# Boese0601/MagicDance

Hardware: NVIDIA H100
Metric: denoise-steps/sec @512x512 50-step DDIM (higher is better)
Workload: dtype f16

## Files before the change

magicdance_b200/csrc/attention.cu:

```cuda
#include <stdlib.h>

#include <type_traits>

#include "common.cuh"

namespace mdb {

constexpr int kBQ = 128;

template <int D, int BKV, int STAGES>
struct AttnCfg {
  static constexpr int kDkChunks = (D + 63) / 64;
  static constexpr int kDV = (D + 15) / 16 * 16;
  static constexpr int kKSteps = kDV / 16;
  static constexpr int kQBytes = kDkChunks * kBQ * 128;
  static constexpr int kKBytes = kDkChunks * BKV * 128;
  static constexpr int kVBytes = kDV * 128;
  static constexpr int kStageBytes = kKBytes + kVBytes;
  static constexpr int kSmem = kQBytes + STAGES * kStageBytes + 1024;
  static_assert(BKV == 64, "one 128-byte swizzle row of keys per V^T tile");
  static_assert(kVBytes % 1024 == 0 && kKBytes % 1024 == 0, "stage tiles start on swizzle-atom boundaries");
};

struct AttnKParams {
  CUtensorMap tmQ, tmK0, tmV0, tmK1, tmV1;
  __half* out;
  long long ldo;
  int nq, n0, n1;
  int kv0_batches, kv1_batches;
  int ldv0_batch, ldv1_batch;
  int bank_batches;
  float scale_log2;
};
struct AttnLseKParams : AttnKParams {
  float* lse;
};

template <int D, int BKV, int STAGES, int MINB, bool LSE = false>
__global__ void __launch_bounds__(kWsThreads, MINB)
    attn_wg_kernel(const __grid_constant__ std::conditional_t<LSE, AttnLseKParams, AttnKParams> p) {
  using C = AttnCfg<D, BKV, STAGES>;
  extern __shared__ uint8_t smem_raw[];
  __shared__ __align__(8) uint64_t q_bar;
  __shared__ __align__(8) uint64_t kv_full[STAGES], kv_empty[STAGES];

  uint8_t* sQ = align1024(smem_raw);
  uint8_t* sKV = sQ + C::kQBytes;

  const int warp = threadIdx.x >> 5;
  const int lane = threadIdx.x & 31;
  const int q0 = blockIdx.x * kBQ;
  const int head = blockIdx.y;
  const int b = blockIdx.z;
  const int t0 = (p.n0 + BKV - 1) / BKV;
  const int t1 = (b < p.bank_batches && p.n1 > 0) ? (p.n1 + BKV - 1) / BKV : 0;
  const int n_tiles = t0 + t1;

  pdl_launch_dependents();
  if (warp == kProducerWarp && lane == 0) {
    tma_prefetch_desc(&p.tmQ);
    tma_prefetch_desc(&p.tmK0);
    tma_prefetch_desc(&p.tmV0);
    mbar_init(&q_bar, 1);
    ring_init<STAGES>(kv_full, kv_empty, 1);
    fence_barrier_init();
  }
  __syncthreads();
  pdl_wait();

  if (warp == kProducerWarp) {
    if (lane == 0) {
      mbar_expect_tx(&q_bar, C::kQBytes);
      for (int dc = 0; dc < C::kDkChunks; ++dc)
        tma_load_3d(sQ + dc * (kBQ * 128), &p.tmQ, &q_bar, dc * 64, head, b * p.nq + q0);
      for (int j = 0; j < n_tiles; ++j) {
        const bool src1 = j >= t0;
        const int key0 = (src1 ? (j - t0) : j) * BKV;
        const CUtensorMap* tk = src1 ? &p.tmK1 : &p.tmK0;
        const CUtensorMap* tv = src1 ? &p.tmV1 : &p.tmV0;
        const int nsrc = src1 ? p.n1 : p.n0;
        const int kvb = src1 ? (p.kv1_batches > 1 ? b : 0) : (p.kv0_batches > 1 ? b : 0);
        const int ldvb = src1 ? p.ldv1_batch : p.ldv0_batch;
        const int s = ring_acquire<STAGES>(kv_empty, j);
        mbar_expect_tx(&kv_full[s], C::kStageBytes);
        uint8_t* sk = sKV + s * C::kStageBytes;
        uint8_t* sv = sk + C::kKBytes;
        for (int dc = 0; dc < C::kDkChunks; ++dc)
          tma_load_3d(sk + dc * (BKV * 128), tk, &kv_full[s], dc * 64, head, kvb * nsrc + key0);
        tma_load_2d(sv, tv, &kv_full[s], kvb * ldvb + key0, head * D);
      }
    }
  } else {
    const int wg = warp >> 2;
    const uint32_t q_addr = smem_u32(sQ) + wg * (64 * 128);
    const int cq = 2 * (lane & 3);
    float o[C::kDV / 2];
#pragma unroll
    for (int i = 0; i < C::kDV / 2; ++i) o[i] = 0.f;
    float m_run[2] = {-INFINITY, -INFINITY};
    float l_run[2] = {0.f, 0.f};
    mbar_wait(&q_bar, 0);

    for (int j = 0; j < n_tiles; ++j) {
      const bool src1 = j >= t0;
      const int key0 = (src1 ? (j - t0) : j) * BKV;
      const int valid = min(BKV, (src1 ? p.n1 : p.n0) - key0);
      const int s = ring_wait_full<STAGES>(kv_full, j);
      const uint32_t k_addr = smem_u32(sKV + s * C::kStageBytes);
      const uint32_t v_addr = k_addr + C::kKBytes;

      float sc[BKV / 2];
      wgmma_fence();
#pragma unroll
      for (int ks = 0; ks < C::kKSteps; ++ks) {
        const int dc = ks >> 2, kk = ks & 3;
        const uint64_t da = wgmma_desc_k_sw128(q_addr + dc * (kBQ * 128)) + 2 * kk;
        const uint64_t db = wgmma_desc_k_sw128(k_addr + dc * (BKV * 128)) + 2 * kk;
        wgmma_ss<BKV>(sc, da, db, ks != 0 ? 1u : 0u);
      }
      wgmma_commit();
      wgmma_wait<0>();
      wgmma_fence_regs(sc);

      if (valid < BKV) {
#pragma unroll
        for (int i = 0; i < BKV / 2; ++i)
          if (8 * (i >> 2) + cq + (i & 1) >= valid) sc[i] = -INFINITY;
      }
      float mx[2] = {-INFINITY, -INFINITY};
#pragma unroll
      for (int i = 0; i < BKV / 2; ++i) mx[(i >> 1) & 1] = fmaxf(mx[(i >> 1) & 1], sc[i]);
      float alpha[2], neg_m[2];
#pragma unroll
      for (int h = 0; h < 2; ++h) {
        mx[h] = fmaxf(mx[h], __shfl_xor_sync(0xffffffffu, mx[h], 1));
        mx[h] = fmaxf(mx[h], __shfl_xor_sync(0xffffffffu, mx[h], 2));
        const float m_new = fmaxf(m_run[h], mx[h] * p.scale_log2);
        alpha[h] = ex2_approx(m_run[h] - m_new);
        m_run[h] = m_new;
        neg_m[h] = -m_new;
      }
      float ls[2] = {0.f, 0.f};
      uint32_t pa[BKV / 16][4];
#pragma unroll
      for (int i = 0; i < BKV / 2; i += 2) {
        const int h = (i >> 1) & 1;
        const float e0 = ex2_approx(fmaf(sc[i], p.scale_log2, neg_m[h]));
        const float e1 = ex2_approx(fmaf(sc[i + 1], p.scale_log2, neg_m[h]));
        ls[h] += e0 + e1;
        pa[i >> 3][(i >> 1) & 3] = pack_half2(e0, e1);
      }
#pragma unroll
      for (int h = 0; h < 2; ++h) l_run[h] = fmaf(l_run[h], alpha[h], ls[h]);
#pragma unroll
      for (int i = 0; i < C::kDV / 2; ++i) o[i] *= alpha[(i >> 1) & 1];

      wgmma_fence();
#pragma unroll
      for (int kk = 0; kk < BKV / 16; ++kk)
        wgmma_rs<C::kDV>(o, pa[kk], wgmma_desc_k_sw128(v_addr) + 2 * kk, 1u);
      wgmma_commit();
      wgmma_wait<0>();
      wgmma_fence_regs(o);
      mbar_arrive(&kv_empty[s]);
    }

    float inv_l[2], l_row[2];
#pragma unroll
    for (int h = 0; h < 2; ++h) {
      float l = l_run[h];
      l += __shfl_xor_sync(0xffffffffu, l, 1);
      l += __shfl_xor_sync(0xffffffffu, l, 2);
      inv_l[h] = 1.0f / l;
      l_row[h] = l;
    }
    const int r = wg * 64 + (warp & 3) * 16 + (lane >> 2);
    if constexpr (LSE) {
      if ((lane & 3) == 0) {
#pragma unroll
        for (int h = 0; h < 2; ++h) {
          const int q = q0 + r + 8 * h;
          if (q < p.nq)
            p.lse[(static_cast<long long>(b) * gridDim.y + head) * p.nq + q] =
                (m_run[h] + log2f(l_row[h])) * 0.6931471805599453f;
        }
      }
    }
#pragma unroll
    for (int h = 0; h < 2; ++h) {
      const int q = q0 + r + 8 * h;
      if (q < p.nq) {
        __half* op = p.out + (static_cast<long long>(b) * p.nq + q) * p.ldo + head * D + cq;
#pragma unroll
        for (int c8 = 0; c8 < D / 8; ++c8)
          *reinterpret_cast<uint32_t*>(op + 8 * c8) =
              pack_half2(o[4 * c8 + 2 * h] * inv_l[h], o[4 * c8 + 2 * h + 1] * inv_l[h]);
      }
    }
  }
}

static int g_attn40_2q_min_ctas = 512;
int get_attn_tuning() { return g_attn40_2q_min_ctas; }
void set_attn_tuning(int v) { g_attn40_2q_min_ctas = v; }

template <int D, int BKV, int STAGES, int MINB, bool LSE = false, typename P>
static int launch_attn(const P& kp, dim3 grid, cudaStream_t st) {
  using C = AttnCfg<D, BKV, STAGES>;
  static_assert(MINB == 1 || C::kSmem <= 113 * 1024, "two CTAs per SM must fit");
  constexpr auto kern = attn_wg_kernel<D, BKV, STAGES, MINB, LSE>;
  if (int rc = set_max_dyn_smem<kern>(C::kSmem)) return rc;
  MDB_CHECK_CUDA(launch_pdl(kern, grid, dim3(kWsThreads), C::kSmem, st, kp));
  count_launch();
  return MDB_OK;
}

template <int D, int BKV>
static int build_and_launch(const mdb_attn_desc* a, float* lse, cudaStream_t st) {
  constexpr int kDV = AttnCfg<D, BKV, 1>::kDV;
  AttnKParams kp;
  memset(&kp, 0, sizeof(kp));
  const int hd = a->heads * a->d;
  int rc;
  if ((rc = tmap_heads(&kp.tmQ, a->q, a->d, a->heads, (uint64_t)a->batch * a->nq, a->ldq, kBQ))) return rc;
  auto mk_kv = [&](const void* k, long long ldk, const void* vt, long long ldvt, int n, int nb, int ldvb,
                   CUtensorMap* tk, CUtensorMap* tv) -> int {
    int r = tmap_heads(tk, k, a->d, a->heads, (uint64_t)nb * n, ldk, BKV);
    if (r) return r;
    return tmap_rows(tv, vt, (uint64_t)nb * ldvb, hd, ldvt, 64, kDV);
  };
  if ((rc = mk_kv(a->k0, a->ldk0, a->vt0, a->ldvt0, a->n0, a->kv0_batches, a->ldv0_batch, &kp.tmK0, &kp.tmV0))) return rc;
  if (a->n1 > 0) {
    if ((rc = mk_kv(a->k1, a->ldk1, a->vt1, a->ldvt1, a->n1, a->kv1_batches, a->ldv1_batch, &kp.tmK1, &kp.tmV1)))
      return rc;
  }
  kp.out = static_cast<__half*>(a->out);
  kp.ldo = a->ldo;
  kp.nq = a->nq;
  kp.n0 = a->n0;
  kp.n1 = a->n1;
  kp.kv0_batches = a->kv0_batches;
  kp.kv1_batches = a->kv1_batches;
  kp.ldv0_batch = a->ldv0_batch;
  kp.ldv1_batch = a->ldv1_batch;
  kp.bank_batches = a->n1 > 0 ? a->bank_batches : 0;
  kp.scale_log2 = a->scale * 1.4426950408889634f;
  dim3 grid((a->nq + kBQ - 1) / kBQ, a->heads, a->batch);
  if (lse != nullptr) {
    AttnLseKParams lp;
    memset(&lp, 0, sizeof(lp));
    static_cast<AttnKParams&>(lp) = kp;
    lp.lse = lse;
    if constexpr (D == 40) {
      const long long ctas = (long long)grid.x * grid.y * grid.z;
      if (ctas >= (long long)g_attn40_2q_min_ctas) return launch_attn<D, BKV, 3, 2, true>(lp, grid, st);
    }
    return launch_attn<D, BKV, (D == 160 ? 2 : 4), 1, true>(lp, grid, st);
  }
  if constexpr (D == 40) {
    const long long ctas = (long long)grid.x * grid.y * grid.z;
    if (ctas >= (long long)g_attn40_2q_min_ctas) return launch_attn<D, BKV, 3, 2>(kp, grid, st);
  }
  return launch_attn<D, BKV, (D == 160 ? 2 : 4), 1>(kp, grid, st);
}

static int attention_entry(const mdb_attn_desc* a, float* lse, cudaStream_t st) {
  switch (a->d) {
    case 40:
      return build_and_launch<40, 64>(a, lse, st);
    case 80:
      return build_and_launch<80, 64>(a, lse, st);
    case 160:
      return build_and_launch<160, 64>(a, lse, st);
    default:
      set_error("mdb_attention_f16: head dim %d not supported (40, 80, 160)", a->d);
      return MDB_ERR_UNSUPPORTED;
  }
}

int attention_check_desc(const mdb_attn_desc* a) {
  MDB_REQUIRE(a != nullptr, "mdb_attention_f16: null descriptor");
  MDB_REQUIRE(a->q && a->k0 && a->vt0 && a->out, "mdb_attention_f16: null operand");
  MDB_REQUIRE(a->batch > 0 && a->heads > 0 && a->nq > 0 && a->n0 > 0 && a->n1 >= 0,
              "mdb_attention_f16: bad shape");
  MDB_REQUIRE(a->n1 == 0 || (a->k1 && a->vt1), "mdb_attention_f16: n1 > 0 needs k1/vt1");
  MDB_REQUIRE(a->kv0_batches == 1 || a->kv0_batches == a->batch, "mdb_attention_f16: kv0_batches must be 1 or batch");
  MDB_REQUIRE(a->n1 == 0 || a->kv1_batches == 1 || a->kv1_batches >= a->bank_batches,
              "mdb_attention_f16: kv1_batches must be 1 or cover bank_batches");
  MDB_REQUIRE(a->ldv0_batch >= a->n0 && a->ldv0_batch % 8 == 0, "mdb_attention_f16: ldv0_batch must be >= n0 and %% 8");
  MDB_REQUIRE(a->ldo % 8 == 0 && (reinterpret_cast<uintptr_t>(a->out) & 15) == 0, "mdb_attention_f16: out alignment");
  return MDB_OK;
}

}

using namespace mdb;

extern "C" int mdb_attention_f16(const mdb_attn_desc* a, mdb_stream_t stream) {
  const int rc = attention_check_desc(a);
  if (rc) return rc;
  return attention_entry(a, nullptr, static_cast<cudaStream_t>(stream));
}

extern "C" int mdb_attention_lse_f16(const mdb_attn_desc* a, float* lse, mdb_stream_t stream) {
  const int rc = attention_check_desc(a);
  if (rc) return rc;
  MDB_REQUIRE(lse != nullptr, "mdb_attention_lse_f16: null lse");
  return attention_entry(a, lse, static_cast<cudaStream_t>(stream));
}
```

magicdance_b200/csrc/common.cuh:

```cuda
#pragma once

#include <cuda.h>
#include <cuda_fp16.h>
#include <cuda_runtime.h>
#include <cudaTypedefs.h>
#include <stdint.h>
#include <stdio.h>
#include <string.h>

#include "../../include/magicdance_b200.h"
#include "wgmma.cuh"

namespace mdb {

void set_error(const char* fmt, ...);

#define MDB_CHECK_CUDA(expr)                                                                     \
  do {                                                                                           \
    cudaError_t _e = (expr);                                                                     \
    if (_e != cudaSuccess) {                                                                     \
      mdb::set_error("%s:%d: %s failed: %s", __FILE__, __LINE__, #expr, cudaGetErrorString(_e)); \
      return MDB_ERR_CUDA;                                                                       \
    }                                                                                            \
  } while (0)

#define MDB_REQUIRE(cond, ...)      \
  do {                              \
    if (!(cond)) {                  \
      mdb::set_error(__VA_ARGS__);  \
      return MDB_ERR_INVALID;       \
    }                               \
  } while (0)

void count_launch(int n = 1);
int get_gemm_tuning(int key);
void set_gemm_tuning(int key, int value);
int get_attn_tuning();
void set_attn_tuning(int v);

constexpr int kNumSms = 132;

int tmap_rows(CUtensorMap* out, const void* base, uint64_t inner, uint64_t rows, long long ld, uint32_t box_inner,
              uint32_t box_rows);
int tmap_heads(CUtensorMap* out, const void* base, int d, int heads, uint64_t tokens, long long ld,
               uint32_t box_tokens);
int tmap_nhwc(CUtensorMap* out, const void* base, int c, int w, int h, int nb, long long ld, const uint32_t box[4],
              int cs);

enum { kBoxOk, kBoxWideRows, kBoxRowsPerTile, kBoxImagesPerTile, kBoxTooLarge };
int pixel_box(int ho, int wo, int cs, int rows, bool fwd, uint32_t box[4]);

#ifdef __CUDACC__

bool pdl_enabled();
template <typename... KArgs, typename... Args>
inline cudaError_t launch_pdl_cluster2(void (*kernel)(KArgs...), dim3 grid, dim3 block, size_t smem,
                                       cudaStream_t stream, unsigned cluster_x, unsigned cluster_z, Args&&... args) {
  cudaLaunchConfig_t cfg;
  memset(&cfg, 0, sizeof(cfg));
  cfg.gridDim = grid;
  cfg.blockDim = block;
  cfg.dynamicSmemBytes = smem;
  cfg.stream = stream;
  cudaLaunchAttribute attr[2];
  int n = 0;
  if (cluster_z > 1 || cluster_x > 1) {
    attr[n].id = cudaLaunchAttributeClusterDimension;
    attr[n].val.clusterDim.x = cluster_x;
    attr[n].val.clusterDim.y = 1;
    attr[n].val.clusterDim.z = cluster_z;
    ++n;
  }
  if (pdl_enabled()) {
    attr[n].id = cudaLaunchAttributeProgrammaticStreamSerialization;
    attr[n].val.programmaticStreamSerializationAllowed = 1;
    ++n;
  }
  cfg.attrs = attr;
  cfg.numAttrs = n;
  return cudaLaunchKernelEx(&cfg, kernel, static_cast<KArgs>(args)...);
}
template <typename... KArgs, typename... Args>
inline cudaError_t launch_pdl_cluster(void (*kernel)(KArgs...), dim3 grid, dim3 block, size_t smem,
                                      cudaStream_t stream, unsigned cluster_z, Args&&... args) {
  return launch_pdl_cluster2(kernel, grid, block, smem, stream, 1u, cluster_z, static_cast<Args&&>(args)...);
}
template <typename... KArgs, typename... Args>
inline cudaError_t launch_pdl(void (*kernel)(KArgs...), dim3 grid, dim3 block, size_t smem, cudaStream_t stream,
                              Args&&... args) {
  return launch_pdl_cluster2(kernel, grid, block, smem, stream, 1u, 1u, static_cast<Args&&>(args)...);
}
template <auto Kernel>
inline int set_max_dyn_smem(int bytes) {
  static bool done = false;
  if (!done) {
    MDB_CHECK_CUDA(cudaFuncSetAttribute(Kernel, cudaFuncAttributeMaxDynamicSharedMemorySize, bytes));
    done = true;
  }
  return MDB_OK;
}

__device__ __forceinline__ uint32_t smem_u32(const void* p) {
  return static_cast<uint32_t>(__cvta_generic_to_shared(p));
}

__device__ __forceinline__ bool elect_one() {
  uint32_t pred = 0;
  asm volatile(
      "{\n\t.reg .pred P;\n\t"
      "elect.sync _|P, 0xffffffff;\n\t"
      "selp.u32 %0, 1, 0, P;\n\t}"
      : "=r"(pred));
  return pred != 0;
}

__device__ __forceinline__ void pdl_launch_dependents() { asm volatile("griddepcontrol.launch_dependents;" ::: "memory"); }
__device__ __forceinline__ void pdl_wait() { asm volatile("griddepcontrol.wait;" ::: "memory"); }

__device__ __forceinline__ void mbar_init(uint64_t* bar, uint32_t count) {
  asm volatile("mbarrier.init.shared::cta.b64 [%0], %1;" ::"r"(smem_u32(bar)), "r"(count));
}
__device__ __forceinline__ void fence_barrier_init() {
  asm volatile("fence.mbarrier_init.release.cluster;" ::: "memory");
}
__device__ __forceinline__ void mbar_expect_tx(uint64_t* bar, uint32_t bytes) {
  asm volatile("mbarrier.arrive.expect_tx.shared::cta.b64 _, [%0], %1;" ::"r"(smem_u32(bar)), "r"(bytes)
               : "memory");
}
__device__ __forceinline__ void mbar_arrive(uint64_t* bar) {
  asm volatile("mbarrier.arrive.shared::cta.b64 _, [%0];" ::"r"(smem_u32(bar)) : "memory");
}
__device__ __forceinline__ void mbar_wait(uint64_t* bar, uint32_t parity) {
  uint32_t addr = smem_u32(bar);
  asm volatile(
      "{\n\t.reg .pred P1;\n\t"
      "WAIT_LOOP:\n\t"
      "mbarrier.try_wait.parity.shared::cta.b64 P1, [%0], %1;\n\t"
      "@P1 bra DONE;\n\t"
      "bra WAIT_LOOP;\n\t"
      "DONE:\n\t}"
      ::"r"(addr), "r"(parity)
      : "memory");
}

constexpr int kConsumers = 256;
constexpr int kProducerWarp = kConsumers / 32;
constexpr int kWsThreads = kConsumers + 32;

__device__ __forceinline__ uint8_t* align1024(uint8_t* p) {
  return reinterpret_cast<uint8_t*>((reinterpret_cast<uintptr_t>(p) + 1023) & ~uintptr_t(1023));
}

template <int S>
__device__ __forceinline__ void ring_init(uint64_t* full, uint64_t* empty, uint32_t full_count) {
  for (int s = 0; s < S; ++s) {
    mbar_init(&full[s], full_count);
    mbar_init(&empty[s], kConsumers);
  }
}
template <int S>
__device__ __forceinline__ int ring_acquire(uint64_t* empty, int it) {
  const int s = it % S;
  mbar_wait(&empty[s], ((it / S) & 1) ^ 1);
  return s;
}
template <int S>
__device__ __forceinline__ int ring_wait_full(uint64_t* full, int it) {
  const int s = it % S;
  mbar_wait(&full[s], (it / S) & 1);
  return s;
}

__device__ __forceinline__ void tma_prefetch_desc(const CUtensorMap* m) {
  asm volatile("prefetch.tensormap [%0];" ::"l"(reinterpret_cast<uint64_t>(m)) : "memory");
}
__device__ __forceinline__ void tma_load_2d(void* dst, const CUtensorMap* m, uint64_t* bar, int c0, int c1) {
  asm volatile(
      "cp.async.bulk.tensor.2d.shared::cluster.global.tile.mbarrier::complete_tx::bytes [%0], [%1, {%3, %4}], [%2];"
      ::"r"(smem_u32(dst)), "l"(reinterpret_cast<uint64_t>(m)), "r"(smem_u32(bar)), "r"(c0), "r"(c1)
      : "memory");
}
__device__ __forceinline__ void tma_load_3d(void* dst, const CUtensorMap* m, uint64_t* bar, int c0, int c1, int c2) {
  asm volatile(
      "cp.async.bulk.tensor.3d.shared::cluster.global.tile.mbarrier::complete_tx::bytes [%0], [%1, {%3, %4, %5}], [%2];"
      ::"r"(smem_u32(dst)), "l"(reinterpret_cast<uint64_t>(m)), "r"(smem_u32(bar)), "r"(c0), "r"(c1), "r"(c2)
      : "memory");
}
__device__ __forceinline__ void tma_load_4d(void* dst, const CUtensorMap* m, uint64_t* bar, int c0, int c1, int c2,
                                            int c3) {
  asm volatile(
      "cp.async.bulk.tensor.4d.shared::cluster.global.tile.mbarrier::complete_tx::bytes [%0], [%1, {%3, %4, %5, %6}], [%2];"
      ::"r"(smem_u32(dst)), "l"(reinterpret_cast<uint64_t>(m)), "r"(smem_u32(bar)), "r"(c0), "r"(c1), "r"(c2), "r"(c3)
      : "memory");
}

__device__ __forceinline__ uint32_t cluster_ctarank() {
  uint32_t r;
  asm volatile("mov.u32 %0, %%cluster_ctarank;" : "=r"(r));
  return r;
}
__device__ __forceinline__ void cluster_sync_all() {
  asm volatile("barrier.cluster.arrive.release.aligned;" ::: "memory");
  asm volatile("barrier.cluster.wait.acquire.aligned;" ::: "memory");
}
__device__ __forceinline__ uint32_t dsmem_map(uint32_t local_smem_addr, uint32_t rank) {
  uint32_t a;
  asm volatile("mapa.shared::cluster.u32 %0, %1, %2;" : "=r"(a) : "r"(local_smem_addr), "r"(rank));
  return a;
}
__device__ __forceinline__ float4 dsmem_ld_f4(uint32_t cluster_addr) {
  float4 v;
  asm volatile("ld.shared::cluster.v4.f32 {%0, %1, %2, %3}, [%4];"
               : "=f"(v.x), "=f"(v.y), "=f"(v.z), "=f"(v.w)
               : "r"(cluster_addr));
  return v;
}

__device__ __forceinline__ void fence_proxy_async_smem() {
  asm volatile("fence.proxy.async.shared::cta;" ::: "memory");
}

__device__ __forceinline__ uint64_t wgmma_desc_k_sw128(uint32_t smem_addr) {
  uint64_t d = 0;
  d |= static_cast<uint64_t>((smem_addr & 0x3FFFF) >> 4);
  d |= static_cast<uint64_t>(1) << 16;
  d |= static_cast<uint64_t>(1024 >> 4) << 32;
  d |= static_cast<uint64_t>(1) << 62;
  return d;
}
__device__ __forceinline__ uint64_t wgmma_desc_mn_sw128(uint32_t smem_addr, uint32_t chunk_bytes) {
  uint64_t d = 0;
  d |= static_cast<uint64_t>((smem_addr & 0x3FFFF) >> 4);
  d |= static_cast<uint64_t>((chunk_bytes >> 4) & 0x3FFF) << 16;
  d |= static_cast<uint64_t>(1024 >> 4) << 32;
  d |= static_cast<uint64_t>(1) << 62;
  return d;
}
__device__ __forceinline__ void wgmma_fence() { asm volatile("wgmma.fence.sync.aligned;" ::: "memory"); }
__device__ __forceinline__ void wgmma_commit() { asm volatile("wgmma.commit_group.sync.aligned;" ::: "memory"); }
template <int N>
__device__ __forceinline__ void wgmma_wait() { asm volatile("wgmma.wait_group.sync.aligned %0;" ::"n"(N) : "memory"); }
template <int R>
__device__ __forceinline__ void wgmma_fence_regs(float (&d)[R]) {
#pragma unroll
  for (int i = 0; i < R; ++i) asm volatile("" : "+f"(d[i])::"memory");
}
__device__ __forceinline__ void named_bar_sync(int id, int threads) {
  asm volatile("bar.sync %0, %1;" ::"r"(id), "r"(threads) : "memory");
}

__device__ __forceinline__ uint32_t pack_half2(float a, float b) {
  __half2 h = __floats2half2_rn(a, b);
  return *reinterpret_cast<uint32_t*>(&h);
}

__device__ __forceinline__ float ex2_approx(float x) {
  float y;
  asm("ex2.approx.ftz.f32 %0, %1;" : "=f"(y) : "f"(x));
  return y;
}
__device__ __forceinline__ float silu_f(float x) { return x / (1.0f + __expf(-x)); }
__device__ __forceinline__ float gelu_erf_f(float x) { return 0.5f * x * (1.0f + erff(x * 0.70710678118654752f)); }
__device__ __forceinline__ float dsilu(float x) {
  const float s = 1.0f / (1.0f + __expf(-x));
  return s * (1.0f + x * (1.0f - s));
}
__device__ __forceinline__ float dgelu_erf(float x) {
  return 0.5f * (1.0f + erff(x * 0.70710678118654752f)) + x * 0.39894228040143268f * __expf(-0.5f * x * x);
}

struct GbOut {
  void* p;
  long long ld;
  int f32, acc;
};

__device__ __forceinline__ void gb_store2(const GbOut& o, long long row, int col, float v0, float v1) {
  if (o.p == nullptr) return;
  if (o.f32) {
    float2* d = reinterpret_cast<float2*>(static_cast<float*>(o.p) + row * o.ld + col);
    if (o.acc) {
      const float2 x = *d;
      v0 += x.x;
      v1 += x.y;
    }
    *d = make_float2(v0, v1);
  } else {
    __half2* d = reinterpret_cast<__half2*>(static_cast<__half*>(o.p) + row * o.ld + col);
    if (o.acc) {
      const float2 x = __half22float2(*d);
      v0 += x.x;
      v1 += x.y;
    }
    *d = __floats2half2_rn(v0, v1);
  }
}
#endif

inline GbOut gb_out(void* p, long long ld, int dtype, int acc) {
  GbOut o;
  o.p = p;
  o.ld = ld;
  o.f32 = dtype == MDB_DTYPE_F32;
  o.acc = acc != 0;
  return o;
}

int launch_colsum_finalize(const float* ws, int n, int segs, int parts, float* out, long long stride, int acc,
                           cudaStream_t st);

}
```

Before: 89.98.

## Add warp-specialized FA3-style pipelined attention kernel for head dim 40

Adds a dedicated head-dim-40 attention kernel with one TMA producer warpgroup and three MMA consumer warpgroups. It uses 128-key tiles, register reallocation via setmaxnreg, and ping-pong named barriers so one warpgroup's QK/PV wgmma overlaps another's softmax. The next tile's QK is issued alongside the previous tile's PV. The kernel is the default path for d=40 whenever there are more than 128 keys, and the tuning knob is repurposed (negative values select the old kernel). It aims to hide softmax latency and raise tensor-core utilization, at the cost of more code, a large register budget, and one CTA per SM.

```diff
diff --git a/magicdance_b200/csrc/attention.cu b/magicdance_b200/csrc/attention.cu
--- a/magicdance_b200/csrc/attention.cu
+++ b/magicdance_b200/csrc/attention.cu
@@ -200,7 +200,236 @@
   }
 }
 
-static int g_attn40_2q_min_ctas = 512;
+struct Attn40Pipe {
+  static constexpr int kBKV = 128;
+  static constexpr int kDV = 48;
+  static constexpr int kKBytes = kBKV * 128;
+  static constexpr int kVAtom = kDV * 128;
+  static constexpr int kStageBytes = kKBytes + 2 * kVAtom;
+  static constexpr int kStages = 3;
+  static constexpr int kProducerRegs = 24;
+  static_assert(kVAtom % 1024 == 0 && kKBytes % 1024 == 0, "stage tiles start on swizzle-atom boundaries");
+};
+template <int NCW>
+struct Attn40PipeShape {
+  static constexpr int kBQ = 64 * NCW;
+  static constexpr int kThreads = 128 * (NCW + 1);
+  static constexpr int kMmaRegs = (65536 / kThreads / 8 * 8 * kThreads - 128 * Attn40Pipe::kProducerRegs) /
+                                  (128 * NCW) / 8 * 8;
+  static constexpr int kSmem = kBQ * 128 + Attn40Pipe::kStages * Attn40Pipe::kStageBytes + 1024;
+};
+
+template <int NCW, bool LSE = false>
+__global__ void __launch_bounds__(Attn40PipeShape<NCW>::kThreads, 1)
+    attn40_pipe_kernel(const __grid_constant__ std::conditional_t<LSE, AttnLseKParams, AttnKParams> p) {
+  using C = Attn40Pipe;
+  using Sh = Attn40PipeShape<NCW>;
+  constexpr int kS = C::kStages;
+  constexpr int kProducer = 128 * NCW;
+  extern __shared__ uint8_t smem_raw[];
+  __shared__ __align__(8) uint64_t q_bar;
+  __shared__ __align__(8) uint64_t kv_full[kS], kv_empty[kS];
+
+  uint8_t* sQ = align1024(smem_raw);
+  uint8_t* sKV = sQ + Sh::kBQ * 128;
+
+  const int warp = threadIdx.x >> 5;
+  const int lane = threadIdx.x & 31;
+  const int wg = warp >> 2;
+  const int q0 = blockIdx.x * Sh::kBQ;
+  const int head = blockIdx.y;
+  const int b = blockIdx.z;
+  const int t0 = (p.n0 + C::kBKV - 1) / C::kBKV;
+  const int t1 = (b < p.bank_batches && p.n1 > 0) ? (p.n1 + C::kBKV - 1) / C::kBKV : 0;
+  const int n_tiles = t0 + t1;
+
+  pdl_launch_dependents();
+  if (threadIdx.x == kProducer) {
+    tma_prefetch_desc(&p.tmQ);
+    tma_prefetch_desc(&p.tmK0);
+    tma_prefetch_desc(&p.tmV0);
+    mbar_init(&q_bar, 1);
+    for (int s = 0; s < kS; ++s) {
+      mbar_init(&kv_full[s], 1);
+      mbar_init(&kv_empty[s], 128 * NCW);
+    }
+    fence_barrier_init();
+  }
+  __syncthreads();
+  pdl_wait();
+
+  if (wg == NCW) {
+    setmaxnreg_dec<C::kProducerRegs>();
+    if (threadIdx.x == kProducer) {
+      mbar_expect_tx(&q_bar, Sh::kBQ * 128);
+      for (int w = 0; w < NCW; ++w) tma_load_3d(sQ + w * (64 * 128), &p.tmQ, &q_bar, 0, head, b * p.nq + q0 + 64 * w);
+      for (int j = 0; j < n_tiles; ++j) {
+        const bool src1 = j >= t0;
+        const int key0 = (src1 ? (j - t0) : j) * C::kBKV;
+        const CUtensorMap* tk = src1 ? &p.tmK1 : &p.tmK0;
+        const CUtensorMap* tv = src1 ? &p.tmV1 : &p.tmV0;
+        const int nsrc = src1 ? p.n1 : p.n0;
+        const int kvb = src1 ? (p.kv1_batches > 1 ? b : 0) : (p.kv0_batches > 1 ? b : 0);
+        const int vcol = kvb * (src1 ? p.ldv1_batch : p.ldv0_batch) + key0;
+        const int s = ring_acquire<kS>(kv_empty, j);
+        mbar_expect_tx(&kv_full[s], C::kStageBytes);
+        uint8_t* sk = sKV + s * C::kStageBytes;
+        tma_load_3d(sk, tk, &kv_full[s], 0, head, kvb * nsrc + key0);
+        tma_load_2d(sk + C::kKBytes, tv, &kv_full[s], vcol, head * 40);
+        tma_load_2d(sk + C::kKBytes + C::kVAtom, tv, &kv_full[s], vcol + 64, head * 40);
+      }
+    }
+  } else {
+    setmaxnreg_inc<Sh::kMmaRegs>();
+    const uint32_t q_addr = smem_u32(sQ) + wg * (64 * 128);
+    const int cq = 2 * (lane & 3);
+    float o[C::kDV / 2];
+#pragma unroll
+    for (int i = 0; i < C::kDV / 2; ++i) o[i] = 0.f;
+    float m_run[2] = {-INFINITY, -INFINITY};
+    float l_run[2] = {0.f, 0.f};
+    float sc[C::kBKV / 2];
+    uint32_t pa[C::kBKV / 16][4];
+
+    auto issue_qk = [&](int s) {
+      const uint32_t k_addr = smem_u32(sKV + s * C::kStageBytes);
+#pragma unroll
+      for (int ks = 0; ks < C::kDV / 16; ++ks)
+        wgmma_ss<C::kBKV>(sc, wgmma_desc_k_sw128(q_addr) + 2 * ks, wgmma_desc_k_sw128(k_addr) + 2 * ks,
+                          ks != 0 ? 1u : 0u);
+    };
+    auto issue_pv = [&](int s) {
+      const uint32_t v_addr = smem_u32(sKV + s * C::kStageBytes) + C::kKBytes;
+#pragma unroll
+      for (int kk = 0; kk < C::kBKV / 16; ++kk)
+        wgmma_rs<C::kDV>(o, pa[kk], wgmma_desc_k_sw128(v_addr + (kk >> 2) * C::kVAtom) + 2 * (kk & 3), 1u);
+    };
+    auto softmax = [&](int j, float (&alpha)[2]) {
+      const bool src1 = j >= t0;
+      const int valid = (src1 ? p.n1 : p.n0) - (src1 ? (j - t0) : j) * C::kBKV;
+      if (valid < C::kBKV) {
+        const int lim = valid - cq;
+#pragma unroll
+        for (int i = 0; i < C::kBKV / 2; ++i)
+          if (8 * (i >> 2) + (i & 1) >= lim) sc[i] = -INFINITY;
+      }
+      float mx[2] = {-INFINITY, -INFINITY};
+#pragma unroll
+      for (int i = 0; i < C::kBKV / 2; ++i) mx[(i >> 1) & 1] = fmaxf(mx[(i >> 1) & 1], sc[i]);
+      float neg_m[2];
+#pragma unroll
+      for (int h = 0; h < 2; ++h) {
+        mx[h] = fmaxf(mx[h], __shfl_xor_sync(0xffffffffu, mx[h], 1));
+        mx[h] = fmaxf(mx[h], __shfl_xor_sync(0xffffffffu, mx[h], 2));
+        const float m_new = fmaxf(m_run[h], mx[h] * p.scale_log2);
+        alpha[h] = ex2_approx(m_run[h] - m_new);
+        m_run[h] = m_new;
+        neg_m[h] = -m_new;
+      }
+      float ls[2] = {0.f, 0.f};
+#pragma unroll
+      for (int i = 0; i < C::kBKV / 2; i += 2) {
+        const int h = (i >> 1) & 1;
+        sc[i] = ex2_approx(fmaf(sc[i], p.scale_log2, neg_m[h]));
+        sc[i + 1] = ex2_approx(fmaf(sc[i + 1], p.scale_log2, neg_m[h]));
+        ls[h] += sc[i] + sc[i + 1];
+      }
+#pragma unroll
+      for (int h = 0; h < 2; ++h) l_run[h] = fmaf(l_run[h], alpha[h], ls[h]);
+    };
+    auto pack_p = [&] {
+#pragma unroll
+      for (int i = 0; i < C::kBKV / 2; i += 2) pa[i >> 3][(i >> 1) & 3] = pack_half2(sc[i], sc[i + 1]);
+    };
+
+    auto turn_begin = [&] { named_bar_sync(1 + wg, 256); };
+    auto turn_end = [&](bool last) {
+      if (!(last && wg == NCW - 1)) named_bar_arrive(1 + (wg + 1) % NCW, 256);
+    };
+    if (wg == NCW - 1) named_bar_arrive(1, 256);
+
+    mbar_wait(&q_bar, 0);
+    int s_prev = ring_wait_full<kS>(kv_full, 0);
+    turn_begin();
+    wgmma_fence();
+    issue_qk(s_prev);
+    wgmma_commit();
+    turn_end(false);
+    wgmma_wait<0>();
+    wgmma_fence_regs(sc);
+    {
+      float alpha[2];
+      softmax(0, alpha);
+      pack_p();
+    }
+    for (int j = 1; j < n_tiles; ++j) {
+      const int s = ring_wait_full<kS>(kv_full, j);
+      turn_begin();
+      wgmma_fence();
+      issue_qk(s);
+      wgmma_commit();
+      issue_pv(s_prev);
+      wgmma_commit();
+      turn_end(false);
+      wgmma_wait<1>();
+      wgmma_fence_regs(sc);
+      float alpha[2];
+      softmax(j, alpha);
+      wgmma_wait<0>();
+      wgmma_fence_regs(o);
+      mbar_arrive(&kv_empty[s_prev]);
+#pragma unroll
+      for (int i = 0; i < C::kDV / 2; ++i) o[i] *= alpha[(i >> 1) & 1];
+      pack_p();
+      s_prev = s;
+    }
+    turn_begin();
+    wgmma_fence();
+    issue_pv(s_prev);
+    wgmma_commit();
+    turn_end(true);
+    wgmma_wait<0>();
+    wgmma_fence_regs(o);
+    mbar_arrive(&kv_empty[s_prev]);
+
+    float inv_l[2], l_row[2];
+#pragma unroll
+    for (int h = 0; h < 2; ++h) {
+      float l = l_run[h];
+      l += __shfl_xor_sync(0xffffffffu, l, 1);
+      l += __shfl_xor_sync(0xffffffffu, l, 2);
+      inv_l[h] = 1.0f / l;
+      l_row[h] = l;
+    }
+    const int r = wg * 64 + (warp & 3) * 16 + (lane >> 2);
+    if constexpr (LSE) {
+      if ((lane & 3) == 0) {
+#pragma unroll
+        for (int h = 0; h < 2; ++h) {
+          const int q = q0 + r + 8 * h;
+          if (q < p.nq)
+            p.lse[(static_cast<long long>(b) * gridDim.y + head) * p.nq + q] =
+                (m_run[h] + log2f(l_row[h])) * 0.6931471805599453f;
+        }
+      }
+    }
+#pragma unroll
+    for (int h = 0; h < 2; ++h) {
+      const int q = q0 + r + 8 * h;
+      if (q < p.nq) {
+        __half* op = p.out + (static_cast<long long>(b) * p.nq + q) * p.ldo + head * 40 + cq;
+#pragma unroll
+        for (int c8 = 0; c8 < 40 / 8; ++c8)
+          *reinterpret_cast<uint32_t*>(op + 8 * c8) =
+              pack_half2(o[4 * c8 + 2 * h] * inv_l[h], o[4 * c8 + 2 * h + 1] * inv_l[h]);
+      }
+    }
+  }
+}
+
+constexpr int kAttn40Consumers = 3;
+
+static int g_attn40_2q_min_ctas = 0;
 int get_attn_tuning() { return g_attn40_2q_min_ctas; }
 void set_attn_tuning(int v) { g_attn40_2q_min_ctas = v; }
 
@@ -215,17 +444,15 @@
   return MDB_OK;
 }
 
-template <int D, int BKV>
-static int build_and_launch(const mdb_attn_desc* a, float* lse, cudaStream_t st) {
-  constexpr int kDV = AttnCfg<D, BKV, 1>::kDV;
-  AttnKParams kp;
+static int attn_params(const mdb_attn_desc* a, uint32_t q_box, uint32_t k_box, AttnKParams& kp) {
+  const int kDV = (a->d + 15) / 16 * 16;
   memset(&kp, 0, sizeof(kp));
   const int hd = a->heads * a->d;
   int rc;
-  if ((rc = tmap_heads(&kp.tmQ, a->q, a->d, a->heads, (uint64_t)a->batch * a->nq, a->ldq, kBQ))) return rc;
+  if ((rc = tmap_heads(&kp.tmQ, a->q, a->d, a->heads, (uint64_t)a->batch * a->nq, a->ldq, q_box))) return rc;
   auto mk_kv = [&](const void* k, long long ldk, const void* vt, long long ldvt, int n, int nb, int ldvb,
                    CUtensorMap* tk, CUtensorMap* tv) -> int {
-    int r = tmap_heads(tk, k, a->d, a->heads, (uint64_t)nb * n, ldk, BKV);
+    int r = tmap_heads(tk, k, a->d, a->heads, (uint64_t)nb * n, ldk, k_box);
     if (r) return r;
     return tmap_rows(tv, vt, (uint64_t)nb * ldvb, hd, ldvt, 64, kDV);
   };
@@ -245,28 +472,67 @@
   kp.ldv1_batch = a->ldv1_batch;
   kp.bank_batches = a->n1 > 0 ? a->bank_batches : 0;
   kp.scale_log2 = a->scale * 1.4426950408889634f;
+  return MDB_OK;
+}
+
+static AttnLseKParams with_lse(const AttnKParams& kp, float* lse) {
+  AttnLseKParams lp;
+  memset(&lp, 0, sizeof(lp));
+  static_cast<AttnKParams&>(lp) = kp;
+  lp.lse = lse;
+  return lp;
+}
+
+template <int D, int BKV>
+static int build_and_launch(const mdb_attn_desc* a, float* lse, cudaStream_t st) {
+  AttnKParams kp;
+  if (int rc = attn_params(a, kBQ, BKV, kp)) return rc;
   dim3 grid((a->nq + kBQ - 1) / kBQ, a->heads, a->batch);
+  const long long ctas = (long long)grid.x * grid.y * grid.z;
+  const bool capped = D == 40 && ctas >= (g_attn40_2q_min_ctas < 0 ? -(long long)g_attn40_2q_min_ctas : 512);
   if (lse != nullptr) {
-    AttnLseKParams lp;
-    memset(&lp, 0, sizeof(lp));
-    static_cast<AttnKParams&>(lp) = kp;
-    lp.lse = lse;
-    if constexpr (D == 40) {
-      const long long ctas = (long long)grid.x * grid.y * grid.z;
-      if (ctas >= (long long)g_attn40_2q_min_ctas) return launch_attn<D, BKV, 3, 2, true>(lp, grid, st);
-    }
+    const AttnLseKParams lp = with_lse(kp, lse);
+    if constexpr (D == 40)
+      if (capped) return launch_attn<D, BKV, 3, 2, true>(lp, grid, st);
     return launch_attn<D, BKV, (D == 160 ? 2 : 4), 1, true>(lp, grid, st);
   }
-  if constexpr (D == 40) {
-    const long long ctas = (long long)grid.x * grid.y * grid.z;
-    if (ctas >= (long long)g_attn40_2q_min_ctas) return launch_attn<D, BKV, 3, 2>(kp, grid, st);
-  }
+  if constexpr (D == 40)
+    if (capped) return launch_attn<D, BKV, 3, 2>(kp, grid, st);
   return launch_attn<D, BKV, (D == 160 ? 2 : 4), 1>(kp, grid, st);
+}
+
+template <int NCW, bool LSE, typename P>
+static int launch_attn40_pipe_kernel(const P& kp, dim3 grid, cudaStream_t st) {
+  using Sh = Attn40PipeShape<NCW>;
+  constexpr auto kern = attn40_pipe_kernel<NCW, LSE>;
+  static int regs = -1;
+  if (regs < 0) {
+    cudaFuncAttributes fa;
+    MDB_CHECK_CUDA(cudaFuncGetAttributes(&fa, kern));
+    regs = fa.numRegs;
+  }
+  MDB_REQUIRE(regs * Sh::kThreads >= 128 * Attn40Pipe::kProducerRegs + 128 * NCW * Sh::kMmaRegs,
+              "attn40_pipe_kernel: compiled to %d registers per thread, too few to raise the MMA warpgroups to %d",
+              regs, Sh::kMmaRegs);
+  if (int rc = set_max_dyn_smem<kern>(Sh::kSmem)) return rc;
+  MDB_CHECK_CUDA(launch_pdl(kern, grid, dim3(Sh::kThreads), Sh::kSmem, st, kp));
+  count_launch();
+  return MDB_OK;
+}
+
+static int launch_attn40_pipe(const mdb_attn_desc* a, float* lse, cudaStream_t st) {
+  constexpr int kBQ40 = Attn40PipeShape<kAttn40Consumers>::kBQ;
+  AttnKParams kp;
+  if (int rc = attn_params(a, 64, Attn40Pipe::kBKV, kp)) return rc;
+  dim3 grid((a->nq + kBQ40 - 1) / kBQ40, a->heads, a->batch);
+  if (lse != nullptr) return launch_attn40_pipe_kernel<kAttn40Consumers, true>(with_lse(kp, lse), grid, st);
+  return launch_attn40_pipe_kernel<kAttn40Consumers, false>(kp, grid, st);
 }
 
 static int attention_entry(const mdb_attn_desc* a, float* lse, cudaStream_t st) {
   switch (a->d) {
     case 40:
+      if (g_attn40_2q_min_ctas >= 0 && a->n0 + a->n1 > Attn40Pipe::kBKV) return launch_attn40_pipe(a, lse, st);
       return build_and_launch<40, 64>(a, lse, st);
     case 80:
       return build_and_launch<80, 64>(a, lse, st);
diff --git a/magicdance_b200/csrc/common.cuh b/magicdance_b200/csrc/common.cuh
--- a/magicdance_b200/csrc/common.cuh
+++ b/magicdance_b200/csrc/common.cuh
@@ -245,8 +245,15 @@
 #pragma unroll
   for (int i = 0; i < R; ++i) asm volatile("" : "+f"(d[i])::"memory");
 }
+template <int R>
+__device__ __forceinline__ void setmaxnreg_dec() { asm volatile("setmaxnreg.dec.sync.aligned.u32 %0;" ::"n"(R)); }
+template <int R>
+__device__ __forceinline__ void setmaxnreg_inc() { asm volatile("setmaxnreg.inc.sync.aligned.u32 %0;" ::"n"(R)); }
 __device__ __forceinline__ void named_bar_sync(int id, int threads) {
   asm volatile("bar.sync %0, %1;" ::"r"(id), "r"(threads) : "memory");
+}
+__device__ __forceinline__ void named_bar_arrive(int id, int threads) {
+  asm volatile("bar.arrive %0, %1;" ::"r"(id), "r"(threads) : "memory");
 }
 
 __device__ __forceinline__ uint32_t pack_half2(float a, float b) {
```

New measurement: 92.30 (median of 6 runs). +2.6%, better.
